# kunpengcompute/media

Hardware: AMD Instinct MI355X
Metric: encoded fps @1080p I420 baseline-profile, 1/2/4/8 MI355X vs OpenH264 CPU (higher is better)
Workload: dtype u8

## Files before the change

### media_amd/csrc/k_deblock.h

```cpp
#pragma once
#include "dev_common.h"

namespace h264 {

__constant__ const uint8_t c_alpha[52] = {0,  0,  0,  0,  0,  0,  0,  0,  0,  0,  0,  0,  0,   0,   0,   0,   4,   4,
                                          5,  6,  7,  8,  9,  10, 12, 13, 15, 17, 20, 22, 25,  28,  32,  36,  40,  45,
                                          50, 56, 63, 71, 80, 90, 101, 113, 127, 144, 162, 182, 203, 226, 255, 255};
__constant__ const uint8_t c_beta[52] = {0,  0,  0,  0,  0,  0,  0,  0,  0,  0,  0,  0,  0,  0,  0,  0,  2,  2,
                                         2,  3,  3,  3,  3,  4,  4,  4,  6,  6,  7,  7,  8,  8,  9,  9,  10, 10,
                                         11, 11, 12, 12, 13, 13, 14, 14, 15, 15, 16, 16, 17, 17, 18, 18};
__constant__ const uint8_t c_tc0[52][3] = {
    {0, 0, 0},   {0, 0, 0},   {0, 0, 0},    {0, 0, 0},    {0, 0, 0},    {0, 0, 0},   {0, 0, 0},   {0, 0, 0},  {0, 0, 0},
    {0, 0, 0},   {0, 0, 0},   {0, 0, 0},    {0, 0, 0},    {0, 0, 0},    {0, 0, 0},   {0, 0, 0},   {0, 0, 0},  {0, 0, 1},
    {0, 0, 1},   {0, 0, 1},   {0, 0, 1},    {0, 1, 1},    {0, 1, 1},    {1, 1, 1},   {1, 1, 1},   {1, 1, 1},  {1, 1, 1},
    {1, 1, 2},   {1, 1, 2},   {1, 1, 2},    {1, 1, 2},    {1, 2, 3},    {1, 2, 3},   {2, 2, 3},   {2, 2, 4},  {2, 3, 4},
    {2, 3, 4},   {3, 3, 5},   {3, 4, 6},    {3, 4, 6},    {4, 5, 7},    {4, 5, 8},   {4, 6, 9},   {5, 7, 10}, {6, 8, 11},
    {6, 8, 13},  {7, 10, 14}, {8, 11, 16},  {9, 12, 18},  {10, 13, 20}, {11, 15, 23}, {13, 17, 25}};

struct DbParams {
    uint8_t* pl[3];
    const MbInfo* mb;
    int cw, ch, mbw, mbh;
    int alpha_y, beta_y, alpha_c, beta_c;
    int tc0_y[3], tc0_c[3];
    SliceRows sl;
    const uint8_t* bs;
    const uint8_t* mbqp;
    int oa, ob;
    int cqo_cb, cqo_cr;
};

__device__ __forceinline__ void filter_line(uint8_t* pix, int xs, int bS, int alpha, int beta, int tc0, bool chroma)
{
    const int p0 = pix[-xs], p1 = pix[-2 * xs], q0 = pix[0], q1 = pix[xs];
    if (iabs(p0 - q0) >= alpha || iabs(p1 - p0) >= beta || iabs(q1 - q0) >= beta) return;
    if (chroma) {
        if (bS < 4) {
            const int tc = tc0 + 1;
            const int d = clip3(-tc, tc, (((q0 - p0) << 2) + (p1 - q1) + 4) >> 3);
            pix[-xs] = (uint8_t)clip255(p0 + d);
            pix[0] = (uint8_t)clip255(q0 - d);
        } else {
            pix[-xs] = (uint8_t)((2 * p1 + p0 + q1 + 2) >> 2);
            pix[0] = (uint8_t)((2 * q1 + q0 + p1 + 2) >> 2);
        }
        return;
    }
    const int p2 = pix[-3 * xs], q2 = pix[2 * xs];
    const int ap = iabs(p2 - p0), aq = iabs(q2 - q0);
    if (bS < 4) {
        const int tc = tc0 + (ap < beta) + (aq < beta);
        const int d = clip3(-tc, tc, (((q0 - p0) << 2) + (p1 - q1) + 4) >> 3);
        pix[-xs] = (uint8_t)clip255(p0 + d);
        pix[0] = (uint8_t)clip255(q0 - d);
        if (ap < beta) pix[-2 * xs] = (uint8_t)(p1 + clip3(-tc0, tc0, (p2 + ((p0 + q0 + 1) >> 1) - (p1 << 1)) >> 1));
        if (aq < beta) pix[xs] = (uint8_t)(q1 + clip3(-tc0, tc0, (q2 + ((p0 + q0 + 1) >> 1) - (q1 << 1)) >> 1));
    } else {
        const int p3 = pix[-4 * xs], q3 = pix[3 * xs];
        const bool strong = iabs(p0 - q0) < ((alpha >> 2) + 2);
        if (ap < beta && strong) {
            pix[-xs] = (uint8_t)((p2 + 2 * p1 + 2 * p0 + 2 * q0 + q1 + 4) >> 3);
            pix[-2 * xs] = (uint8_t)((p2 + p1 + p0 + q0 + 2) >> 2);
            pix[-3 * xs] = (uint8_t)((2 * p3 + 3 * p2 + p1 + p0 + q0 + 4) >> 3);
        } else pix[-xs] = (uint8_t)((2 * p1 + p0 + q1 + 2) >> 2);
        if (aq < beta && strong) {
            pix[0] = (uint8_t)((p1 + 2 * p0 + 2 * q0 + 2 * q1 + q2 + 4) >> 3);
            pix[xs] = (uint8_t)((p0 + q0 + q1 + q2 + 2) >> 2);
            pix[2 * xs] = (uint8_t)((2 * q3 + 3 * q2 + q1 + q0 + p0 + 4) >> 3);
        } else pix[0] = (uint8_t)((2 * q1 + q0 + p1 + 2) >> 2);
    }
}

enum { DB_LP = 24, DB_CP = 12 };

__global__ __launch_bounds__(64) void k_deblock_diag(DbParams D, int s)
{
    const int lane = threadIdx.x;
    const int ymin = max(0, (s - (D.mbw - 1) + 1) >> 1);
    const int my = ymin + blockIdx.x, mx = s - 2 * my;
    if (my >= D.mbh || mx < 0 || mx >= D.mbw) return;
    const int cs = D.cw / 2;
    __shared__ __attribute__((aligned(16))) uint8_t s_y[20 * DB_LP];
    __shared__ __attribute__((aligned(16))) uint8_t s_c[2][10 * DB_CP];
    __shared__ uint8_t s_bs[2][16];

    for (int i = lane; i < 20 * 5; i += 64) {
        const int r = i / 5, c = i - r * 5;
        const int gy = 16 * my - 4 + r, gx = 16 * mx - 4 + c * 4;
        uint32_t v = 0;
        if (gy >= 0 && gx >= 0) v = *(const uint32_t*)(D.pl[0] + (size_t)gy * D.cw + gx);
        *(uint32_t*)(s_y + r * DB_LP + c * 4) = v;
    }
    for (int i = lane; i < 2 * 10 * 5; i += 64) {
        const int pl = i / 50, k = i - pl * 50, r = k / 5, c = k - r * 5;
        const int gy = 8 * my - 2 + r, gx = 8 * mx - 2 + c * 2;
        uint16_t v = 0;
        if (gy >= 0 && gx >= 0) v = *(const uint16_t*)(D.pl[1 + pl] + (size_t)gy * cs + gx);
        *(uint16_t*)(s_c[pl] + r * DB_CP + c * 2) = v;
    }
    if (lane < 32) {
        const int dir = lane >> 4, e = (lane >> 2) & 3, k = lane & 3;
        const int bS = D.bs[((size_t)my * D.mbw + mx) * 32 + lane];
        s_bs[dir][e * 4 + k] = (uint8_t)bS;
    }
    __syncthreads();

    const bool isY = lane < 16, isC = lane >= 16 && lane < 32;
    const int cpl = (lane >> 3) & 1, cl = lane & 7;
#pragma unroll 1
    for (int dir = 0; dir < 2; dir++) {
#pragma unroll 1
        for (int e = 0; e < 4; e++) {
            if (isY) {
                const int bS = s_bs[dir][e * 4 + (lane >> 2)];
                if (bS) {
                    uint8_t* p = dir == 0 ? s_y + (4 + lane) * DB_LP + 4 + 4 * e : s_y + (4 + 4 * e) * DB_LP + 4 + lane;
                    filter_line(p, dir == 0 ? 1 : DB_LP, bS, D.alpha_y, D.beta_y, bS < 4 ? D.tc0_y[bS - 1] : 0, false);
                }
            } else if (isC && !(e & 1)) {
                const int bS = s_bs[dir][e * 4 + (cl >> 1)];
                if (bS) {
                    uint8_t* p = dir == 0 ? s_c[cpl] + (2 + cl) * DB_CP + 2 + 2 * e : s_c[cpl] + (2 + 2 * e) * DB_CP + 2 + cl;
                    filter_line(p, dir == 0 ? 1 : DB_CP, bS, D.alpha_c, D.beta_c, bS < 4 ? D.tc0_c[bS - 1] : 0, true);
                }
            }
            __syncthreads();
        }
    }
    for (int i = lane; i < 20 * 5; i += 64) {
        const int r = i / 5, c = i - r * 5;
        const int gy = 16 * my - 4 + r, gx = 16 * mx - 4 + c * 4;
        if (gy < 0 || gx < 0) continue;
        if (r < 4 && c == 0) continue;
        *(uint32_t*)(D.pl[0] + (size_t)gy * D.cw + gx) = *(const uint32_t*)(s_y + r * DB_LP + c * 4);
    }
    for (int i = lane; i < 2 * 10 * 5; i += 64) {
        const int pl = i / 50, k = i - pl * 50, r = k / 5, c = k - r * 5;
        const int gy = 8 * my - 2 + r, gx = 8 * mx - 2 + c * 2;
        if (gy < 0 || gx < 0) continue;
        if (r < 2 && c == 0) continue;
        *(uint16_t*)(D.pl[1 + pl] + (size_t)gy * cs + gx) = *(const uint16_t*)(s_c[pl] + r * DB_CP + c * 2);
    }
}

typedef unsigned long long u64;
#define AT_LOAD(p) __hip_atomic_load((p), __ATOMIC_RELAXED, __HIP_MEMORY_SCOPE_AGENT)
#define AT_STORE(p, v) __hip_atomic_store((p), (v), __ATOMIC_RELAXED, __HIP_MEMORY_SCOPE_AGENT)

struct DbRowParams {
    DbParams d;
    u64* handoff;
    const uint32_t* bs;
    unsigned* err;
    unsigned serial;
    const unsigned* anybs;
    const unsigned* anypcm;
    const unsigned* anyintra;
    unsigned pic_serial;
    int npic;
    int need_intra;
    size_t st_y, st_c, st_handoff;
    int st_mb;
    int row0;
    const uint32_t* itemtab;
    size_t st_ring_y, st_ring_c;
};

template <bool BS4>
__device__ __forceinline__ void filt_uni(const int p3, int& p2, int& p1, int& p0, int& q0, int& q1, int& q2, const int q3,
                                         int bS, bool chroma, int alpha, int beta, int t1, int t2, int t3)
{
    const int tc0 = bS == 1 ? t1 : (bS == 2 ? t2 : t3);
    const int fm = -(int)(bS != 0 && iabs(p0 - q0) < alpha && iabs(p1 - p0) < beta && iabs(q1 - q0) < beta);
    const int lum = chroma ? 0 : -1;
    const int apm = lum & -(int)(iabs(p2 - p0) < beta), aqm = lum & -(int)(iabs(q2 - q0) < beta);
    const int tc = tc0 + (chroma ? 1 : 0) - apm - aqm;
    const int d = clip3(-tc, tc, (((q0 - p0) << 2) + (p1 - q1) + 4) >> 3);
    const int avg = (p0 + q0 + 1) >> 1;
    int dp0 = clip255(p0 + d) - p0, dq0 = clip255(q0 - d) - q0;
    int dp1 = apm & clip3(-tc0, tc0, (p2 + avg - (p1 << 1)) >> 1);
    int dq1 = aqm & clip3(-tc0, tc0, (q2 + avg - (q1 << 1)) >> 1);
    int dp2 = 0, dq2 = 0;
    if (BS4) {
        const int s4 = -(int)(bS == 4);
        const int strong = -(int)(iabs(p0 - q0) < ((alpha >> 2) + 2));
        const int sp = apm & strong, sq = aqm & strong;
        const int wp0 = (sp & (((p2 + 2 * p1 + 2 * p0 + 2 * q0 + q1 + 4) >> 3) - p0)) | (~sp & (((2 * p1 + p0 + q1 + 2) >> 2) - p0));
        const int wq0 = (sq & (((p1 + 2 * p0 + 2 * q0 + 2 * q1 + q2 + 4) >> 3) - q0)) | (~sq & (((2 * q1 + q0 + p1 + 2) >> 2) - q0));
        const int wp1 = sp & (((p2 + p1 + p0 + q0 + 2) >> 2) - p1), wq1 = sq & (((p0 + q0 + q1 + q2 + 2) >> 2) - q1);
        const int wp2 = sp & (((2 * p3 + 3 * p2 + p1 + p0 + q0 + 4) >> 3) - p2), wq2 = sq & (((2 * q3 + 3 * q2 + q1 + q0 + p0 + 4) >> 3) - q2);
        dp0 = (s4 & wp0) | (~s4 & dp0); dq0 = (s4 & wq0) | (~s4 & dq0);
        dp1 = (s4 & wp1) | (~s4 & dp1); dq1 = (s4 & wq1) | (~s4 & dq1);
        dp2 = s4 & wp2; dq2 = s4 & wq2;
    }
    p0 += fm & dp0; q0 += fm & dq0; p1 += fm & dp1; q1 += fm & dq1;
    if (BS4) { p2 += fm & dp2; q2 += fm & dq2; }
}

enum { DR_LP = 40, DR_CP = 24 };
#ifdef MI355X_AB_OLD_DB_TILE
enum { DR_CB = 4 * 200, DR_CPS = 4 * 120, DR_TILE = DR_CB + 2 * DR_CPS + 12 };
#else
enum { DR_CB = 4 * 201, DR_CPS = 4 * 144, DR_TILE = DR_CB + 2 * DR_CPS + 12 };
#endif

template <bool BS4, bool PERMB, bool IND>
__device__ __forceinline__ void deblock_rows_picture(const DbRowParams& R, const int pos)
{
    const int bitem = batch_item<IND>(R.itemtab, pos);
    if (R.anybs[bitem] != R.serial) return;
    if (R.anypcm[bitem] == R.pic_serial) return;
    if (R.need_intra != 0 && (R.anyintra[bitem] == R.pic_serial) != (R.need_intra > 0)) return;
    DbParams D = R.d;
    {
        const size_t g = (size_t)bitem;
        D.pl[0] += g * R.st_y; D.pl[1] += g * R.st_c; D.pl[2] += g * R.st_c; D.mb += g * R.st_mb;
        if constexpr (IND) {
            const ItemRef it = item_ref(R.itemtab, pos);
            D.pl[0] += (size_t)it.cur * R.st_ring_y; D.pl[1] += (size_t)it.cur * R.st_ring_c; D.pl[2] += (size_t)it.cur * R.st_ring_c;
            const int qpc = c_chroma_qp[it.qp];
            D.alpha_y = c_alpha[it.qp]; D.beta_y = c_beta[it.qp]; D.alpha_c = c_alpha[qpc]; D.beta_c = c_beta[qpc];
#pragma unroll
            for (int i = 0; i < 3; i++) { D.tc0_y[i] = c_tc0[it.qp][i]; D.tc0_c[i] = c_tc0[qpc][i]; }
        }
        if (PERMB) D.mbqp += g * R.st_mb;
    }
    u64* const handoff = R.handoff + (size_t)bitem * R.st_handoff;
    const uint32_t* const bsw = R.bs + (size_t)bitem * R.st_mb * 8;
    const int lane = threadIdx.x, my = R.row0 + blockIdx.x, cs = D.cw / 2;
    const bool first_row = !D.sl.has_top(my);
    const bool last_row = my == D.mbh - 1 || !D.sl.has_top(my + 1);
    __shared__ __attribute__((aligned(16))) uint8_t s_y[DR_TILE];
#define SY(r, c) s_y[((r) + 4) * DR_LP + (c) + 16]
#define SC(pl, r, c) s_y[DR_CB + (pl) * DR_CPS + ((r) + 4) * DR_CP + (c) + 8]
    bool timed_out = false;
    const int yr = lane >> 2, yc4 = (lane & 3) * 4;
    const int cpl_l = (lane >> 4) & 1, cr_l = (lane >> 1) & 7, cc4 = (lane & 1) * 4;
    const int gk = lane;
    const bool isC = lane >= 16;
    const int fpl = (lane >> 3) & 1, fln = isC ? (lane & 7) : lane;
    const int seg8 = 8 * (isC ? (fln >> 1) : (fln >> 2));
    int al = isC ? D.alpha_c : D.alpha_y, be = isC ? D.beta_c : D.beta_y;
    int t1 = isC ? D.tc0_c[0] : D.tc0_y[0], t2 = isC ? D.tc0_c[1] : D.tc0_y[1], t3 = isC ? D.tc0_c[2] : D.tc0_y[2];
    int alL = al, beL = be, t1L = t1, t2L = t2, t3L = t3, alT = al, beT = be, t1T = t1, t2T = t2, t3T = t3;
    __shared__ uint32_t s_tA[PERMB ? 52 : 1];
    __shared__ uint8_t s_tB[PERMB ? 52 : 1], s_cq[PERMB ? 52 : 1];
    if (PERMB) {
        if (lane < 52) {
            s_tA[lane] = ((uint32_t)c_alpha[lane] << 24) | ((uint32_t)c_tc0[lane][2] << 16) | ((uint32_t)c_tc0[lane][1] << 8) | (uint32_t)c_tc0[lane][0];
            s_tB[lane] = c_beta[lane];
            s_cq[lane] = c_chroma_qp[lane];
        }
        wave_sync();
    }
    const int cqo = fpl ? D.cqo_cr : D.cqo_cb;
    auto thresholds = [&](const int qa, const int qb, int& A, int& B, int& T1, int& T2, int& T3) {
        const int ca = (int)s_cq[clip3(0, 51, qa + cqo)], cb = (int)s_cq[clip3(0, 51, qb + cqo)];
        const int av = ((isC ? ca : qa) + (isC ? cb : qb) + 1) >> 1;
        const uint32_t w = s_tA[clip3(0, 51, av + D.oa)];
        A = (int)(w >> 24); T1 = (int)(w & 255u); T2 = (int)((w >> 8) & 255u); T3 = (int)((w >> 16) & 255u);
        B = (int)s_tB[clip3(0, 51, av + D.ob)];
    };
    uint32_t pf_q = 0;
    int qp_left = 0;
    uint8_t* vrow = isC ? &SC(fpl, fln, -4) : &SY(fln, -4);
    uint8_t* hcol = isC ? &SC(fpl, -4, fln) : &SY(-4, fln);
    const int hstride = isC ? DR_CP : DR_LP;

    uint32_t pf_y = 0, pf_c = 0;
    uint4 pf_b0 = {0, 0, 0, 0}, pf_b1 = pf_b0;
    u64 pf_g = 0;
    const int grow = first_row ? my : my - 1;
    const int glane = lane < 24 ? lane : lane - 24 < 24 ? lane - 24 : lane - 48;
    auto prefetch = [&](int mx) {
        pf_y = *(const uint32_t*)(D.pl[0] + (size_t)(16 * my + yr) * D.cw + 16 * mx + yc4);
        pf_c = *(const uint32_t*)((cpl_l ? D.pl[2] : D.pl[1]) + (size_t)(8 * my + cr_l) * cs + 8 * mx + cc4);
        const uint4* b = (const uint4*)(bsw + ((size_t)my * D.mbw + mx) * 8);
        pf_b0 = b[0]; pf_b1 = b[1];
        pf_g = AT_LOAD(handoff + ((size_t)grow * D.mbw + mx) * 24 + glane);
        if (PERMB) pf_q = (uint32_t)D.mbqp[(size_t)my * D.mbw + mx] | ((uint32_t)D.mbqp[(size_t)grow * D.mbw + mx] << 8);
    };
    auto consume = [&]() {
        asm volatile("" : "+v"(pf_y), "+v"(pf_c), "+v"(pf_g));
        asm volatile("" : "+v"(pf_b0.x), "+v"(pf_b0.y), "+v"(pf_b0.z), "+v"(pf_b0.w));
        asm volatile("" : "+v"(pf_b1.x), "+v"(pf_b1.y), "+v"(pf_b1.z), "+v"(pf_b1.w));
        if (PERMB) asm volatile("" : "+v"(pf_q));
    };
    prefetch(0);
    consume();
    uint32_t cur_y = pf_y, cur_c = pf_c, cur_q = pf_q;
    uint4 b0 = pf_b0, b1 = pf_b1;
    u64 g = pf_g;

    auto store_prev = [&](const int mx, const bool have_cur) {
        if (mx > 0) {
            const int pmx = mx - 1;
            const int co = have_cur ? -16 : 0, cco = have_cur ? -8 : 0;
            const int nrow = last_row ? 16 : 12, ncrow = last_row ? 8 : 6;
            if (yr < nrow) *(uint32_t*)(D.pl[0] + (size_t)(16 * my + yr) * D.cw + 16 * pmx + yc4) = *(const uint32_t*)&SY(yr, co + yc4);
            if (lane < 32 && cr_l < ncrow)
                *(uint32_t*)((cpl_l ? D.pl[2] : D.pl[1]) + (size_t)(8 * my + cr_l) * cs + 8 * pmx + cc4) = *(const uint32_t*)&SC(cpl_l, cr_l, cco + cc4);
            if (!last_row && lane < 24) {
                uint32_t v;
                if (lane < 16) v = *(const uint32_t*)&SY(12 + (gk >> 2), co + (gk & 3) * 4);
                else v = *(const uint32_t*)&SC((gk - 16) >> 2, 6 + (((gk - 16) >> 1) & 1), cco + ((gk - 16) & 1) * 4);
                AT_STORE(handoff + ((size_t)my * D.mbw + pmx) * 24 + gk, ((u64)R.serial << 32) | v);
            }
        }
    };
    for (int mx = 0; mx <= D.mbw; mx++) {
        const bool have_cur = mx < D.mbw;
        if (have_cur) {
            if (mx > 0) {
                *(uint32_t*)&SY(yr, yc4 - 16) = *(const uint32_t*)&SY(yr, yc4);
                if (lane < 32) *(uint32_t*)&SC(cpl_l, cr_l, cc4 - 8) = *(const uint32_t*)&SC(cpl_l, cr_l, cc4);
            }
            wave_sync();
            *(uint32_t*)&SY(yr, yc4) = cur_y;
            if (lane < 32) *(uint32_t*)&SC(cpl_l, cr_l, cc4) = cur_c;
            if (!first_row) {
                unsigned spins = 0;
                while (!timed_out) {
                    const bool bad = lane < 24 && (unsigned)(g >> 32) != R.serial;
                    if (__ballot(bad) == 0ull) break;
                    if (++spins > (1u << 20)) { timed_out = true; break; }
                    __builtin_amdgcn_s_sleep(1);
                    g = AT_LOAD(handoff + ((size_t)grow * D.mbw + mx) * 24 + glane);
                }
                if (lane < 16) *(uint32_t*)&SY(-4 + (gk >> 2), (gk & 3) * 4) = (uint32_t)g;
                else if (lane < 24) *(uint32_t*)&SC((gk - 16) >> 2, -2 + (((gk - 16) >> 1) & 1), ((gk - 16) & 1) * 4) = (uint32_t)g;
            }
            if (mx + 1 < D.mbw) prefetch(mx + 1);
            if (PERMB) {
                const int qc = (int)(cur_q & 255u), qt = (int)(cur_q >> 8);
                thresholds(qc, qc, al, be, t1, t2, t3);
                thresholds(mx > 0 ? qp_left : qc, qc, alL, beL, t1L, t2L, t3L);
                thresholds(qt, qc, alT, beT, t1T, t2T, t3T);
                qp_left = qc;
            }
            wave_sync();
            const bool any_v = (b0.x | b0.y | b0.z | b0.w) != 0, any_h = (b1.x | b1.y | b1.z | b1.w) != 0;
            if (any_v && lane < 32) {
                int px[20];
#pragma unroll
                for (int w = 0; w < 5; w++) {
                    const uint32_t v = *(const uint32_t*)(vrow + 4 * w);
#pragma unroll
                    for (int b = 0; b < 4; b++) px[4 * w + b] = (int)((v >> (8 * b)) & 255);
                }
                const int e0 = (int)(((isC ? b0.x : b0.x) >> seg8) & 255), e1 = (int)(((isC ? b0.z : b0.y) >> seg8) & 255);
                const int e2 = isC ? 0 : (int)((b0.z >> seg8) & 255), e3 = isC ? 0 : (int)((b0.w >> seg8) & 255);
                if (__ballot(e0 != 0) != 0ull) filt_uni<BS4>(px[0], px[1], px[2], px[3], px[4], px[5], px[6], px[7], e0, isC, alL, beL, t1L, t2L, t3L);
                if (__ballot(e1 != 0) != 0ull) filt_uni<BS4>(px[4], px[5], px[6], px[7], px[8], px[9], px[10], px[11], e1, isC, al, be, t1, t2, t3);
                if (__ballot(e2 != 0) != 0ull) filt_uni<BS4>(px[8], px[9], px[10], px[11], px[12], px[13], px[14], px[15], e2, isC, al, be, t1, t2, t3);
                if (__ballot(e3 != 0) != 0ull) filt_uni<BS4>(px[12], px[13], px[14], px[15], px[16], px[17], px[18], px[19], e3, isC, al, be, t1, t2, t3);
#pragma unroll
                for (int w = 0; w < 5; w++)
                    if (w < 3 || !isC)
                        *(uint32_t*)(vrow + 4 * w) = (uint32_t)px[4 * w] | ((uint32_t)px[4 * w + 1] << 8) | ((uint32_t)px[4 * w + 2] << 16) | ((uint32_t)px[4 * w + 3] << 24);
            }
            wave_sync();
            store_prev(mx, true);
            if (any_h && lane < 32) {
                int px[20];
#pragma unroll
                for (int r = 0; r < 20; r++) px[r] = hcol[r * hstride];
                const int e0 = (int)((b1.x >> seg8) & 255), e1 = (int)(((isC ? b1.z : b1.y) >> seg8) & 255);
                const int e2 = isC ? 0 : (int)((b1.z >> seg8) & 255), e3 = isC ? 0 : (int)((b1.w >> seg8) & 255);
                if (__ballot(e0 != 0) != 0ull) filt_uni<BS4>(px[0], px[1], px[2], px[3], px[4], px[5], px[6], px[7], e0, isC, alT, beT, t1T, t2T, t3T);
                if (__ballot(e1 != 0) != 0ull) filt_uni<BS4>(px[4], px[5], px[6], px[7], px[8], px[9], px[10], px[11], e1, isC, al, be, t1, t2, t3);
                if (__ballot(e2 != 0) != 0ull) filt_uni<BS4>(px[8], px[9], px[10], px[11], px[12], px[13], px[14], px[15], e2, isC, al, be, t1, t2, t3);
                if (__ballot(e3 != 0) != 0ull) filt_uni<BS4>(px[12], px[13], px[14], px[15], px[16], px[17], px[18], px[19], e3, isC, al, be, t1, t2, t3);
#pragma unroll
                for (int r = 1; r < 19; r++) {
                    const bool both = r == 3 || r == 4 || r == 7 || r == 8;
                    if (both || !isC) hcol[r * hstride] = (uint8_t)px[r];
                }
            }
            wave_sync();
            consume();
            if (!first_row) {
                if (lane < 16) *(uint32_t*)(D.pl[0] + (size_t)(16 * my - 4 + (gk >> 2)) * D.cw + 16 * mx + (gk & 3) * 4) = *(const uint32_t*)&SY(-4 + (gk >> 2), (gk & 3) * 4);
                else if (lane < 24) {
                    const int k = gk - 16, pl = k >> 2, r = (k >> 1) & 1, c4 = (k & 1) * 4;
                    *(uint32_t*)((pl ? D.pl[2] : D.pl[1]) + (size_t)(8 * my - 2 + r) * cs + 8 * mx + c4) = *(const uint32_t*)&SC(pl, -2 + r, c4);
                }
            }
        }
        if (!have_cur) store_prev(mx, false);
        cur_y = pf_y; cur_c = pf_c; b0 = pf_b0; b1 = pf_b1; g = pf_g; cur_q = pf_q;
        wave_sync();
    }
    if (timed_out && lane == 0) *R.err = 1u;
#undef SY
#undef SC
}
template <bool BS4, bool PERMB = false, bool IND = false>
__global__ __launch_bounds__(64) void k_deblock_rows(DbRowParams R)
{
    __builtin_amdgcn_s_setprio(3);
    for (int pos = blockIdx.y; pos < R.npic; pos += gridDim.y) deblock_rows_picture<BS4, PERMB, IND>(R, pos);
}


template <bool BS4, bool IND>
__device__ __forceinline__ void deblock_pairs_picture(const DbRowParams& R, const int pos)
{
    const int bitem = batch_item<IND>(R.itemtab, pos);
    if (R.anybs[bitem] != R.serial) return;
    if (R.anypcm[bitem] == R.pic_serial) return;
    if (R.need_intra != 0 && (R.anyintra[bitem] == R.pic_serial) != (R.need_intra > 0)) return;
    DbParams D = R.d;
    {
        const size_t g = (size_t)bitem;
        D.pl[0] += g * R.st_y; D.pl[1] += g * R.st_c; D.pl[2] += g * R.st_c; D.mb += g * R.st_mb;
        if constexpr (IND) {
            const ItemRef it = item_ref(R.itemtab, pos);
            D.pl[0] += (size_t)it.cur * R.st_ring_y; D.pl[1] += (size_t)it.cur * R.st_ring_c; D.pl[2] += (size_t)it.cur * R.st_ring_c;
            const int qpc = c_chroma_qp[it.qp];
            D.alpha_y = c_alpha[it.qp]; D.beta_y = c_beta[it.qp]; D.alpha_c = c_alpha[qpc]; D.beta_c = c_beta[qpc];
#pragma unroll
            for (int i = 0; i < 3; i++) { D.tc0_y[i] = c_tc0[it.qp][i]; D.tc0_c[i] = c_tc0[qpc][i]; }
        }
    }
    u64* const handoff = R.handoff + (size_t)bitem * R.st_handoff;
    const uint32_t* const bsw = R.bs + (size_t)bitem * R.st_mb * 8;
    const int lane = threadIdx.x, half = lane >> 5, hl = lane & 31, cs = D.cw / 2;
    const int rowA = R.row0 + 2 * (int)blockIdx.x, rowB = rowA + 1;
    const bool hasB = rowB < D.mbh;
    const int my = half ? (hasB ? rowB : rowA) : rowA;
    const bool live = half == 0 || hasB;
    const bool first_row = half == 0 && rowA == 0;
    const bool last_row = my == D.mbh - 1;
    const bool from_lds = half == 1;
    __shared__ __attribute__((aligned(16))) uint8_t s_yy[2][(DR_TILE + 127) / 128 * 128];
    __shared__ __attribute__((aligned(16))) uint32_t s_ring[2][24];
    uint8_t* const s_y = s_yy[half];
#define SY(r, c) s_y[((r) + 4) * DR_LP + (c) + 16]
#define SC(pl, r, c) s_y[DR_CB + (pl) * DR_CPS + ((r) + 4) * DR_CP + (c) + 8]
    bool timed_out = false;
    const int yr0 = hl >> 2, yc4 = (hl & 3) * 4;
    const int cpl_l = (hl >> 4) & 1, cr_l = (hl >> 1) & 7, cc4 = (hl & 1) * 4;
    const int gk = hl;
    const bool isC = hl >= 16;
    const int fpl = (hl >> 3) & 1, fln = isC ? (hl & 7) : hl;
    const int seg8 = 8 * (isC ? (fln >> 1) : (fln >> 2));
    const int al = isC ? D.alpha_c : D.alpha_y, be = isC ? D.beta_c : D.beta_y;
    const int t1 = isC ? D.tc0_c[0] : D.tc0_y[0], t2 = isC ? D.tc0_c[1] : D.tc0_y[1], t3 = isC ? D.tc0_c[2] : D.tc0_y[2];
    uint8_t* vrow = isC ? &SC(fpl, fln, -4) : &SY(fln, -4);
    uint8_t* hcol = isC ? &SC(fpl, -4, fln) : &SY(-4, fln);
    const int hstride = isC ? DR_CP : DR_LP;

    uint32_t pf_y0 = 0, pf_y1 = 0, pf_c = 0;
    uint4 pf_b0 = {0, 0, 0, 0}, pf_b1 = pf_b0;
    u64 pf_g = 0;
    const int grow = (first_row || half == 1) ? rowA : rowA - 1;
    const int glane = hl < 24 ? hl : hl - 24;
    const int last_mx = D.mbw - 1;
    auto prefetch = [&](int mx) {
        pf_y0 = *(const uint32_t*)(D.pl[0] + (size_t)(16 * my + yr0) * D.cw + 16 * mx + yc4);
        pf_y1 = *(const uint32_t*)(D.pl[0] + (size_t)(16 * my + yr0 + 8) * D.cw + 16 * mx + yc4);
        pf_c = *(const uint32_t*)((cpl_l ? D.pl[2] : D.pl[1]) + (size_t)(8 * my + cr_l) * cs + 8 * mx + cc4);
        const uint4* b = (const uint4*)(bsw + ((size_t)my * D.mbw + mx) * 8);
        pf_b0 = b[0]; pf_b1 = b[1];
        pf_g = AT_LOAD(handoff + ((size_t)grow * D.mbw + mx) * 24 + glane);
    };
    auto consume = [&]() {
        asm volatile("" : "+v"(pf_y0), "+v"(pf_y1), "+v"(pf_c), "+v"(pf_g));
        asm volatile("" : "+v"(pf_b0.x), "+v"(pf_b0.y), "+v"(pf_b0.z), "+v"(pf_b0.w));
        asm volatile("" : "+v"(pf_b1.x), "+v"(pf_b1.y), "+v"(pf_b1.z), "+v"(pf_b1.w));
    };
    prefetch(0);
    consume();
    uint32_t cur_y0 = pf_y0, cur_y1 = pf_y1, cur_c = pf_c;
    uint4 b0 = pf_b0, b1 = pf_b1;
    u64 g = pf_g;

    auto store_prev = [&](const int mx, const bool have_cur) {
        if (mx > 0 && live) {
            const int pmx = mx - 1;
            const int co = have_cur ? -16 : 0, cco = have_cur ? -8 : 0;
            const int nrow = last_row ? 16 : 12, ncrow = last_row ? 8 : 6;
            *(uint32_t*)(D.pl[0] + (size_t)(16 * my + yr0) * D.cw + 16 * pmx + yc4) = *(const uint32_t*)&SY(yr0, co + yc4);
            if (yr0 + 8 < nrow) *(uint32_t*)(D.pl[0] + (size_t)(16 * my + yr0 + 8) * D.cw + 16 * pmx + yc4) = *(const uint32_t*)&SY(yr0 + 8, co + yc4);
            if (cr_l < ncrow)
                *(uint32_t*)((cpl_l ? D.pl[2] : D.pl[1]) + (size_t)(8 * my + cr_l) * cs + 8 * pmx + cc4) = *(const uint32_t*)&SC(cpl_l, cr_l, cco + cc4);
            if (!last_row && hl < 24) {
                uint32_t v;
                if (hl < 16) v = *(const uint32_t*)&SY(12 + (gk >> 2), co + (gk & 3) * 4);
                else v = *(const uint32_t*)&SC((gk - 16) >> 2, 6 + (((gk - 16) >> 1) & 1), cco + ((gk - 16) & 1) * 4);
                if (half == 0) s_ring[pmx & 1][gk] = v;
                else AT_STORE(handoff + ((size_t)my * D.mbw + pmx) * 24 + gk, ((u64)R.serial << 32) | v);
            }
        }
    };
    for (int t = 0; t <= D.mbw + 2; t++) {
        const int mx = t - 2 * half;
        const bool in_range = mx >= 0 && mx <= D.mbw && live;
        const bool have_cur = in_range && mx < D.mbw;
        if (have_cur) {
            if (mx > 0) {
                *(uint32_t*)&SY(yr0, yc4 - 16) = *(const uint32_t*)&SY(yr0, yc4);
                *(uint32_t*)&SY(yr0 + 8, yc4 - 16) = *(const uint32_t*)&SY(yr0 + 8, yc4);
                *(uint32_t*)&SC(cpl_l, cr_l, cc4 - 8) = *(const uint32_t*)&SC(cpl_l, cr_l, cc4);
            }
        }
        wave_sync();
        if (have_cur) {
            *(uint32_t*)&SY(yr0, yc4) = cur_y0;
            *(uint32_t*)&SY(yr0 + 8, yc4) = cur_y1;
            *(uint32_t*)&SC(cpl_l, cr_l, cc4) = cur_c;
        }
        {
            const bool need_g = have_cur && !from_lds && !first_row;
            unsigned spins = 0;
            while (!timed_out) {
                const bool bad = need_g && hl < 24 && (unsigned)(g >> 32) != R.serial;
                if (__ballot(bad) == 0ull) break;
                if (++spins > (1u << 20)) { timed_out = true; break; }
                __builtin_amdgcn_s_sleep(1);
                if (need_g) g = AT_LOAD(handoff + ((size_t)grow * D.mbw + mx) * 24 + glane);
            }
            if (have_cur && !first_row && hl < 24) {
                const uint32_t v = from_lds ? s_ring[mx & 1][gk] : (uint32_t)g;
                if (hl < 16) *(uint32_t*)&SY(-4 + (gk >> 2), (gk & 3) * 4) = v;
                else *(uint32_t*)&SC((gk - 16) >> 2, -2 + (((gk - 16) >> 1) & 1), ((gk - 16) & 1) * 4) = v;
            }
        }
        {
            const int nx = mx + 1 < 0 ? 0 : (mx + 1 > last_mx ? last_mx : mx + 1);
            prefetch(nx);
        }
        wave_sync();
        const bool any_v = have_cur && (b0.x | b0.y | b0.z | b0.w) != 0, any_h = have_cur && (b1.x | b1.y | b1.z | b1.w) != 0;
        if (any_v) {
            int px[20];
#pragma unroll
            for (int w = 0; w < 5; w++) {
                const uint32_t v = *(const uint32_t*)(vrow + 4 * w);
#pragma unroll
                for (int b = 0; b < 4; b++) px[4 * w + b] = (int)((v >> (8 * b)) & 255);
            }
            const int e0 = (int)((b0.x >> seg8) & 255), e1 = (int)(((isC ? b0.z : b0.y) >> seg8) & 255);
            const int e2 = isC ? 0 : (int)((b0.z >> seg8) & 255), e3 = isC ? 0 : (int)((b0.w >> seg8) & 255);
            if (__ballot(e0 != 0) != 0ull) filt_uni<BS4>(px[0], px[1], px[2], px[3], px[4], px[5], px[6], px[7], e0, isC, al, be, t1, t2, t3);
            if (__ballot(e1 != 0) != 0ull) filt_uni<BS4>(px[4], px[5], px[6], px[7], px[8], px[9], px[10], px[11], e1, isC, al, be, t1, t2, t3);
            if (__ballot(e2 != 0) != 0ull) filt_uni<BS4>(px[8], px[9], px[10], px[11], px[12], px[13], px[14], px[15], e2, isC, al, be, t1, t2, t3);
            if (__ballot(e3 != 0) != 0ull) filt_uni<BS4>(px[12], px[13], px[14], px[15], px[16], px[17], px[18], px[19], e3, isC, al, be, t1, t2, t3);
#pragma unroll
            for (int w = 0; w < 5; w++)
                if (w < 3 || !isC)
                    *(uint32_t*)(vrow + 4 * w) = (uint32_t)px[4 * w] | ((uint32_t)px[4 * w + 1] << 8) | ((uint32_t)px[4 * w + 2] << 16) | ((uint32_t)px[4 * w + 3] << 24);
        }
        wave_sync();
        if (have_cur) store_prev(mx, true);
        if (any_h) {
            int px[20];
#pragma unroll
            for (int r = 0; r < 20; r++) px[r] = hcol[r * hstride];
            const int e0 = (int)((b1.x >> seg8) & 255), e1 = (int)(((isC ? b1.z : b1.y) >> seg8) & 255);
            const int e2 = isC ? 0 : (int)((b1.z >> seg8) & 255), e3 = isC ? 0 : (int)((b1.w >> seg8) & 255);
            if (__ballot(e0 != 0) != 0ull) filt_uni<BS4>(px[0], px[1], px[2], px[3], px[4], px[5], px[6], px[7], e0, isC, al, be, t1, t2, t3);
            if (__ballot(e1 != 0) != 0ull) filt_uni<BS4>(px[4], px[5], px[6], px[7], px[8], px[9], px[10], px[11], e1, isC, al, be, t1, t2, t3);
            if (__ballot(e2 != 0) != 0ull) filt_uni<BS4>(px[8], px[9], px[10], px[11], px[12], px[13], px[14], px[15], e2, isC, al, be, t1, t2, t3);
            if (__ballot(e3 != 0) != 0ull) filt_uni<BS4>(px[12], px[13], px[14], px[15], px[16], px[17], px[18], px[19], e3, isC, al, be, t1, t2, t3);
#pragma unroll
            for (int r = 1; r < 19; r++) {
                const bool both = r == 3 || r == 4 || r == 7 || r == 8;
                if (both || !isC) hcol[r * hstride] = (uint8_t)px[r];
            }
        }
        wave_sync();
        consume();
        if (have_cur && !first_row) {
            if (hl < 16) *(uint32_t*)(D.pl[0] + (size_t)(16 * my - 4 + (gk >> 2)) * D.cw + 16 * mx + (gk & 3) * 4) = *(const uint32_t*)&SY(-4 + (gk >> 2), (gk & 3) * 4);
            else if (hl < 24) {
                const int k = gk - 16, pl = k >> 2, r = (k >> 1) & 1, c4 = (k & 1) * 4;
                *(uint32_t*)((pl ? D.pl[2] : D.pl[1]) + (size_t)(8 * my - 2 + r) * cs + 8 * mx + c4) = *(const uint32_t*)&SC(pl, -2 + r, c4);
            }
        }
        if (in_range && !have_cur) store_prev(mx, false);
        if (mx + 1 >= 0 && mx + 1 <= last_mx) { cur_y0 = pf_y0; cur_y1 = pf_y1; cur_c = pf_c; b0 = pf_b0; b1 = pf_b1; g = pf_g; }
        wave_sync();
    }
    if (timed_out && lane == 0) *R.err = 1u;
#undef SY
#undef SC
}
template <bool BS4, bool IND = false>
__global__ __launch_bounds__(64) void k_deblock_pairs(DbRowParams R)
{
    __builtin_amdgcn_s_setprio(3);
    for (int pos = blockIdx.y; pos < R.npic; pos += gridDim.y) deblock_pairs_picture<BS4, IND>(R, pos);
}

}
```

Measured before the change: 26530.

## Run vertical-edge deblocking before waiting on the upper-row handoff

In both deblock kernels, the vertical-edge filtering of the current macroblock is moved ahead of the spin-wait for the row above. The left edge is filtered and written first so the previous macroblock can be stored early, then the interior edges run while the upper row's handoff data may still be arriving. The pair kernel's diagonal stagger is also cut from two macroblocks to one, shortening the pipeline skew between paired rows. This hides inter-row synchronization latency, but depends on vertical filtering never touching the halo rows delivered by the handoff and on the shorter skew being enough to respect horizontal-edge dependencies.

```diff
diff --git a/media_amd/csrc/k_deblock.h b/media_amd/csrc/k_deblock.h
--- a/media_amd/csrc/k_deblock.h
+++ b/media_amd/csrc/k_deblock.h
@@ -318,6 +318,45 @@
             wave_sync();
             *(uint32_t*)&SY(yr, yc4) = cur_y;
             if (lane < 32) *(uint32_t*)&SC(cpl_l, cr_l, cc4) = cur_c;
+            if (mx + 1 < D.mbw) prefetch(mx + 1);
+            if (PERMB) {
+                const int qc = (int)(cur_q & 255u), qt = (int)(cur_q >> 8);
+                thresholds(qc, qc, al, be, t1, t2, t3);
+                thresholds(mx > 0 ? qp_left : qc, qc, alL, beL, t1L, t2L, t3L);
+                thresholds(qt, qc, alT, beT, t1T, t2T, t3T);
+                qp_left = qc;
+            }
+            wave_sync();
+            const bool any_v = (b0.x | b0.y | b0.z | b0.w) != 0, any_h = (b1.x | b1.y | b1.z | b1.w) != 0;
+            const bool v_on = any_v && lane < 32;
+            int px[20];
+            int e1 = 0, e2 = 0, e3 = 0;
+            if (v_on) {
+#pragma unroll
+                for (int w = 0; w < 5; w++) {
+                    const uint32_t v = *(const uint32_t*)(vrow + 4 * w);
+#pragma unroll
+                    for (int b = 0; b < 4; b++) px[4 * w + b] = (int)((v >> (8 * b)) & 255);
+                }
+                const int e0 = (int)((b0.x >> seg8) & 255);
+                e1 = (int)(((isC ? b0.z : b0.y) >> seg8) & 255);
+                e2 = isC ? 0 : (int)((b0.z >> seg8) & 255); e3 = isC ? 0 : (int)((b0.w >> seg8) & 255);
+                if (__ballot(e0 != 0) != 0ull) {
+                    filt_uni<BS4>(px[0], px[1], px[2], px[3], px[4], px[5], px[6], px[7], e0, isC, alL, beL, t1L, t2L, t3L);
+                    *(uint32_t*)vrow = (uint32_t)px[0] | ((uint32_t)px[1] << 8) | ((uint32_t)px[2] << 16) | ((uint32_t)px[3] << 24);
+                }
+            }
+            wave_sync();
+            store_prev(mx, true);
+            if (v_on) {
+                if (__ballot(e1 != 0) != 0ull) filt_uni<BS4>(px[4], px[5], px[6], px[7], px[8], px[9], px[10], px[11], e1, isC, al, be, t1, t2, t3);
+                if (__ballot(e2 != 0) != 0ull) filt_uni<BS4>(px[8], px[9], px[10], px[11], px[12], px[13], px[14], px[15], e2, isC, al, be, t1, t2, t3);
+                if (__ballot(e3 != 0) != 0ull) filt_uni<BS4>(px[12], px[13], px[14], px[15], px[16], px[17], px[18], px[19], e3, isC, al, be, t1, t2, t3);
+#pragma unroll
+                for (int w = 1; w < 5; w++)
+                    if (w < 3 || !isC)
+                        *(uint32_t*)(vrow + 4 * w) = (uint32_t)px[4 * w] | ((uint32_t)px[4 * w + 1] << 8) | ((uint32_t)px[4 * w + 2] << 16) | ((uint32_t)px[4 * w + 3] << 24);
+            }
             if (!first_row) {
                 unsigned spins = 0;
                 while (!timed_out) {
@@ -330,37 +369,7 @@
                 if (lane < 16) *(uint32_t*)&SY(-4 + (gk >> 2), (gk & 3) * 4) = (uint32_t)g;
                 else if (lane < 24) *(uint32_t*)&SC((gk - 16) >> 2, -2 + (((gk - 16) >> 1) & 1), ((gk - 16) & 1) * 4) = (uint32_t)g;
             }
-            if (mx + 1 < D.mbw) prefetch(mx + 1);
-            if (PERMB) {
-                const int qc = (int)(cur_q & 255u), qt = (int)(cur_q >> 8);
-                thresholds(qc, qc, al, be, t1, t2, t3);
-                thresholds(mx > 0 ? qp_left : qc, qc, alL, beL, t1L, t2L, t3L);
-                thresholds(qt, qc, alT, beT, t1T, t2T, t3T);
-                qp_left = qc;
-            }
             wave_sync();
-            const bool any_v = (b0.x | b0.y | b0.z | b0.w) != 0, any_h = (b1.x | b1.y | b1.z | b1.w) != 0;
-            if (any_v && lane < 32) {
-                int px[20];
-#pragma unroll
-                for (int w = 0; w < 5; w++) {
-                    const uint32_t v = *(const uint32_t*)(vrow + 4 * w);
-#pragma unroll
-                    for (int b = 0; b < 4; b++) px[4 * w + b] = (int)((v >> (8 * b)) & 255);
-                }
-                const int e0 = (int)(((isC ? b0.x : b0.x) >> seg8) & 255), e1 = (int)(((isC ? b0.z : b0.y) >> seg8) & 255);
-                const int e2 = isC ? 0 : (int)((b0.z >> seg8) & 255), e3 = isC ? 0 : (int)((b0.w >> seg8) & 255);
-                if (__ballot(e0 != 0) != 0ull) filt_uni<BS4>(px[0], px[1], px[2], px[3], px[4], px[5], px[6], px[7], e0, isC, alL, beL, t1L, t2L, t3L);
-                if (__ballot(e1 != 0) != 0ull) filt_uni<BS4>(px[4], px[5], px[6], px[7], px[8], px[9], px[10], px[11], e1, isC, al, be, t1, t2, t3);
-                if (__ballot(e2 != 0) != 0ull) filt_uni<BS4>(px[8], px[9], px[10], px[11], px[12], px[13], px[14], px[15], e2, isC, al, be, t1, t2, t3);
-                if (__ballot(e3 != 0) != 0ull) filt_uni<BS4>(px[12], px[13], px[14], px[15], px[16], px[17], px[18], px[19], e3, isC, al, be, t1, t2, t3);
-#pragma unroll
-                for (int w = 0; w < 5; w++)
-                    if (w < 3 || !isC)
-                        *(uint32_t*)(vrow + 4 * w) = (uint32_t)px[4 * w] | ((uint32_t)px[4 * w + 1] << 8) | ((uint32_t)px[4 * w + 2] << 16) | ((uint32_t)px[4 * w + 3] << 24);
-            }
-            wave_sync();
-            store_prev(mx, true);
             if (any_h && lane < 32) {
                 int px[20];
 #pragma unroll
@@ -494,8 +503,8 @@
             }
         }
     };
-    for (int t = 0; t <= D.mbw + 2; t++) {
-        const int mx = t - 2 * half;
+    for (int t = 0; t <= D.mbw + 1; t++) {
+        const int mx = t - half;
         const bool in_range = mx >= 0 && mx <= D.mbw && live;
         const bool have_cur = in_range && mx < D.mbw;
         if (have_cur) {
@@ -511,6 +520,41 @@
             *(uint32_t*)&SY(yr0 + 8, yc4) = cur_y1;
             *(uint32_t*)&SC(cpl_l, cr_l, cc4) = cur_c;
         }
+        {
+            const int nx = mx + 1 < 0 ? 0 : (mx + 1 > last_mx ? last_mx : mx + 1);
+            prefetch(nx);
+        }
+        wave_sync();
+        const bool any_v = have_cur && (b0.x | b0.y | b0.z | b0.w) != 0, any_h = have_cur && (b1.x | b1.y | b1.z | b1.w) != 0;
+        int px[20];
+        int e1 = 0, e2 = 0, e3 = 0;
+        if (any_v) {
+#pragma unroll
+            for (int w = 0; w < 5; w++) {
+                const uint32_t v = *(const uint32_t*)(vrow + 4 * w);
+#pragma unroll
+                for (int b = 0; b < 4; b++) px[4 * w + b] = (int)((v >> (8 * b)) & 255);
+            }
+            const int e0 = (int)((b0.x >> seg8) & 255);
+            e1 = (int)(((isC ? b0.z : b0.y) >> seg8) & 255);
+            e2 = isC ? 0 : (int)((b0.z >> seg8) & 255); e3 = isC ? 0 : (int)((b0.w >> seg8) & 255);
+            if (__ballot(e0 != 0) != 0ull) {
+                filt_uni<BS4>(px[0], px[1], px[2], px[3], px[4], px[5], px[6], px[7], e0, isC, al, be, t1, t2, t3);
+                *(uint32_t*)vrow = (uint32_t)px[0] | ((uint32_t)px[1] << 8) | ((uint32_t)px[2] << 16) | ((uint32_t)px[3] << 24);
+            }
+        }
+        wave_sync();
+        if (in_range) store_prev(mx, have_cur);
+        if (any_v) {
+            if (__ballot(e1 != 0) != 0ull) filt_uni<BS4>(px[4], px[5], px[6], px[7], px[8], px[9], px[10], px[11], e1, isC, al, be, t1, t2, t3);
+            if (__ballot(e2 != 0) != 0ull) filt_uni<BS4>(px[8], px[9], px[10], px[11], px[12], px[13], px[14], px[15], e2, isC, al, be, t1, t2, t3);
+            if (__ballot(e3 != 0) != 0ull) filt_uni<BS4>(px[12], px[13], px[14], px[15], px[16], px[17], px[18], px[19], e3, isC, al, be, t1, t2, t3);
+#pragma unroll
+            for (int w = 1; w < 5; w++)
+                if (w < 3 || !isC)
+                    *(uint32_t*)(vrow + 4 * w) = (uint32_t)px[4 * w] | ((uint32_t)px[4 * w + 1] << 8) | ((uint32_t)px[4 * w + 2] << 16) | ((uint32_t)px[4 * w + 3] << 24);
+        }
+        wave_sync();
         {
             const bool need_g = have_cur && !from_lds && !first_row;
             unsigned spins = 0;
@@ -527,33 +571,7 @@
                 else *(uint32_t*)&SC((gk - 16) >> 2, -2 + (((gk - 16) >> 1) & 1), ((gk - 16) & 1) * 4) = v;
             }
         }
-        {
-            const int nx = mx + 1 < 0 ? 0 : (mx + 1 > last_mx ? last_mx : mx + 1);
-            prefetch(nx);
-        }
-        wave_sync();
-        const bool any_v = have_cur && (b0.x | b0.y | b0.z | b0.w) != 0, any_h = have_cur && (b1.x | b1.y | b1.z | b1.w) != 0;
-        if (any_v) {
-            int px[20];
-#pragma unroll
-            for (int w = 0; w < 5; w++) {
-                const uint32_t v = *(const uint32_t*)(vrow + 4 * w);
-#pragma unroll
-                for (int b = 0; b < 4; b++) px[4 * w + b] = (int)((v >> (8 * b)) & 255);
-            }
-            const int e0 = (int)((b0.x >> seg8) & 255), e1 = (int)(((isC ? b0.z : b0.y) >> seg8) & 255);
-            const int e2 = isC ? 0 : (int)((b0.z >> seg8) & 255), e3 = isC ? 0 : (int)((b0.w >> seg8) & 255);
-            if (__ballot(e0 != 0) != 0ull) filt_uni<BS4>(px[0], px[1], px[2], px[3], px[4], px[5], px[6], px[7], e0, isC, al, be, t1, t2, t3);
-            if (__ballot(e1 != 0) != 0ull) filt_uni<BS4>(px[4], px[5], px[6], px[7], px[8], px[9], px[10], px[11], e1, isC, al, be, t1, t2, t3);
-            if (__ballot(e2 != 0) != 0ull) filt_uni<BS4>(px[8], px[9], px[10], px[11], px[12], px[13], px[14], px[15], e2, isC, al, be, t1, t2, t3);
-            if (__ballot(e3 != 0) != 0ull) filt_uni<BS4>(px[12], px[13], px[14], px[15], px[16], px[17], px[18], px[19], e3, isC, al, be, t1, t2, t3);
-#pragma unroll
-            for (int w = 0; w < 5; w++)
-                if (w < 3 || !isC)
-                    *(uint32_t*)(vrow + 4 * w) = (uint32_t)px[4 * w] | ((uint32_t)px[4 * w + 1] << 8) | ((uint32_t)px[4 * w + 2] << 16) | ((uint32_t)px[4 * w + 3] << 24);
-        }
-        wave_sync();
-        if (have_cur) store_prev(mx, true);
+        wave_sync();
         if (any_h) {
             int px[20];
 #pragma unroll
@@ -579,7 +597,6 @@
                 *(uint32_t*)((pl ? D.pl[2] : D.pl[1]) + (size_t)(8 * my - 2 + r) * cs + 8 * mx + c4) = *(const uint32_t*)&SC(pl, -2 + r, c4);
             }
         }
-        if (in_range && !have_cur) store_prev(mx, false);
         if (mx + 1 >= 0 && mx + 1 <= last_mx) { cur_y0 = pf_y0; cur_y1 = pf_y1; cur_c = pf_c; b0 = pf_b0; b1 = pf_b1; g = pf_g; }
         wave_sync();
     }
```

Result: faster. 27420 (median of 6 runs) (+3.4%).
